# kkrt-labs/stwo-brainfuck

Hardware: AMD Instinct MI355X
Metric: trace cells committed+proved/sec (higher is better)
Workload: dtype u32 (M31 / QM31 modular arithmetic)

## Files before the change

bindings/rust/bfhip_sys.rs:

```rust
#![allow(non_camel_case_types, dead_code)]
use std::ffi::{c_char, c_void};

#[repr(C)] pub struct BfhipCtx { _private: [u8; 0] }
#[repr(C)] pub struct BfhipTrace { _private: [u8; 0] }
#[repr(C)] #[derive(Clone, Copy, Default, Debug, PartialEq, Eq)] pub struct BfhipConventions { pub merkle_node_hash: u32, pub mix_u64: u32, pub logup_mask_order: u32, pub merkle_channel: u32, pub reserved: [u32; 4] }
#[repr(C)] #[derive(Clone, Copy, Debug, PartialEq, Eq)] pub struct BfhipPcsConfig { pub pow_bits: u32, pub log_blowup_factor: u32, pub log_last_layer_degree_bound: u32, pub n_queries: u32, pub reserved: [u32; 4] }
#[repr(C)] #[derive(Clone, Copy, Default, Debug, PartialEq, Eq)] pub struct BfhipCheckReport { pub component: u32, pub log_size: u32, pub n_bad_cells: u64, pub first_bad_cell: u64, pub first_bad_constraint: i32, pub first_bad_value: [u32; 4], pub bad_per_constraint: [u64; 16], pub claimed_sum: [u32; 4], pub reserved: [u32; 3] }
#[repr(C)] pub struct BfhipLocalGroup { _private: [u8; 0] }
#[repr(C)] pub struct BfhipPool { _private: [u8; 0] }

#[link(name = "bfhip")]
extern "C" {
    pub fn bfhip_last_error() -> *const c_char;
    pub fn bfhip_device_count() -> i32;
    pub fn bfhip_device_memory(device_id: i32, free_bytes: *mut u64, total_bytes: *mut u64) -> i32;
    pub fn bfhip_ctx_create(device_id: i32, max_log_domain: u32, out: *mut *mut BfhipCtx) -> i32;
    pub fn bfhip_ctx_destroy(ctx: *mut BfhipCtx) -> i32;
    pub fn bfhip_ctx_sync(ctx: *mut BfhipCtx) -> i32;
    pub fn bfhip_ctx_set_overlap(ctx: *mut BfhipCtx, mask: u32) -> i32;
    pub fn bfhip_ctx_memory(ctx: *mut BfhipCtx, out: *mut u64) -> i32;
    pub fn bfhip_ctx_set_sync_policy(ctx: *mut BfhipCtx, blocking: i32) -> i32;
    pub fn bfhip_ctx_set_mailbox(ctx: *mut BfhipCtx, mode: i32, timeout_ms: u32, test_delay_ms: i32) -> i32;
    pub fn bfhip_ctx_set_conventions(ctx: *mut BfhipCtx, conv: *const BfhipConventions) -> i32;
    pub fn bfhip_ctx_get_conventions(ctx: *mut BfhipCtx, out: *mut BfhipConventions) -> i32;
// ... 7 lines not shown
    pub fn bfhip_twiddles(ctx: *mut BfhipCtx, tw_d: *mut *const u32, itw_d: *mut *const u32, root_log: *mut u32) -> i32;
    pub fn bfhip_interpolate(ctx: *mut BfhipCtx, src_cols_h: *const *mut u32, dst_cols_h: *const *mut u32, n_cols: u32, log_size: u32, replicated: i32) -> i32;
    pub fn bfhip_evaluate(ctx: *mut BfhipCtx, coeff_cols_h: *const *mut u32, dst_cols_h: *const *mut u32, n_cols: u32, log_size: u32, log_eval: u32, replicated: i32) -> i32;
    pub fn bfhip_is_first_coeffs(ctx: *mut BfhipCtx, log_min: u32, log_max: u32, dst_cols_h: *const *mut u32) -> i32;
    pub fn bfhip_broadcast16(ctx: *mut BfhipCtx, rows_d: *const u32, dst_d: *mut u32, n_rows: usize) -> i32;
    pub fn bfhip_bit_reverse(ctx: *mut BfhipCtx, src_d: *const u32, dst_d: *mut u32, log_size: u32) -> i32;
    pub fn bfhip_batch_inverse_m31(ctx: *mut BfhipCtx, src_d: *const u32, dst_d: *mut u32, n: usize) -> i32;
    pub fn bfhip_batch_inverse_qm31(ctx: *mut BfhipCtx, src_d: *const *const u32, dst_d: *const *mut u32, n: usize) -> i32;
    pub fn bfhip_accumulate(ctx: *mut BfhipCtx, dst_d: *mut u32, src_d: *const u32, n: usize) -> i32;
    pub fn bfhip_eval_at_point(ctx: *mut BfhipCtx, coeffs_d: *const u32, log_size: u32, replicated: i32, point_h: *const u32, out_h: *mut u32) -> i32;
    pub fn bfhip_merkle_commit_layer(ctx: *mut BfhipCtx, log_size: u32, prev_layer_d: *const c_void, cols_h: *const *const u32, col_shifts_h: *const u32, n_cols: u32, out_hashes_d: *mut c_void) -> i32;
    pub fn bfhip_merkle_commit_layer_poseidon252(ctx: *mut BfhipCtx, log_size: u32, prev_layer_d: *const c_void, cols_h: *const *const u32, col_shifts_h: *const u32, n_cols: u32, out_hashes_d: *mut c_void) -> i32;
    pub fn bfhip_hades_permutation(ctx: *mut BfhipCtx, in_h: *const u32, out_h: *mut u32) -> i32;
    pub fn bfhip_fold_line(ctx: *mut BfhipCtx, src_d: *const *const u32, dst_d: *const *mut u32, log_size: u32, alpha_h: *const u32) -> i32;
    pub fn bfhip_fold_circle_into_line(ctx: *mut BfhipCtx, dst_d: *const *mut u32, src_d: *const *const u32, log_size: u32, alpha_h: *const u32) -> i32;
    pub fn bfhip_grind(ctx: *mut BfhipCtx, digest_h: *const u8, pow_bits: u32, nonce: *mut u64) -> i32;
    pub fn bfhip_gather(ctx: *mut BfhipCtx, col_d: *const u32, idx_h: *const u64, n: usize, out_h: *mut u32) -> i32;
    pub fn bfhip_component_shape(component: i32, n_main_cols: *mut u32, n_logup_cols: *mut u32, n_constraints: *mut u32) -> i32;
    pub fn bfhip_logup_generate(ctx: *mut BfhipCtx, component: i32, log_size: u32, main_rows_h: *const *const u32, lookup_h: *const u32, out_cols_h: *const *mut u32, claimed_sum_h: *mut u32) -> i32;
    pub fn bfhip_eval_constraints(ctx: *mut BfhipCtx, component: i32, log_size: u32, is_first_d: *const u32, main_lde_h: *const *const u32, main_shifts_h: *const u32, inter_lde_h: *const *const u32, inter_shifts_h: *const u32, lookup_h: *const u32, claimed_sum_h: *const u32, coeffs_h: *const u32, acc_d: *const *mut u32) -> i32;
    pub fn bfhip_check_constraints(ctx: *mut BfhipCtx, component: i32, log_size: u32, main_rows_h: *const *const u32, logup_cols_h: *const *const u32, lookup_h: *const u32, claimed_sum_h: *const u32, out: *mut BfhipCheckReport) -> i32;
    pub fn bfhip_accumulate_quotients(ctx: *mut BfhipCtx, log_size: u32, cols_h: *const *const u32, col_shifts_h: *const u32, n_cols: u32, n_samples_h: *const u32, sample_points_h: *const u32, sample_values_h: *const u32, random_coeff_h: *const u32, out_d: *const *mut u32) -> i32;
    pub fn bfhip_prove_brainfuck(ctx: *mut BfhipCtx, code: *const c_char, input_h: *const u8, n_input: usize, log_max_rows: u32, proof_json: *mut *mut c_char, proof_len: *mut usize, transcript: *mut *mut c_char, phase_seconds: *mut f64) -> i32;
    pub fn bfhip_free_host(p: *mut c_void);
    pub fn bfhip_ctx_last_proof_flags(ctx: *mut BfhipCtx, flags: *mut u32) -> i32;
    pub fn bfhip_local_group_create(count: u32, out: *mut *mut BfhipLocalGroup) -> i32;
    pub fn bfhip_local_group_destroy(group: *mut BfhipLocalGroup) -> i32;
    pub fn bfhip_ctx_join_local_group(ctx: *mut BfhipCtx, group: *mut BfhipLocalGroup, rank: u32) -> i32;
    pub fn bfhip_rccl_unique_id(id: *mut u8) -> i32;
    pub fn bfhip_ctx_join_rccl_group(ctx: *mut BfhipCtx, id: *const u8, rank: u32, count: u32) -> i32;
// ... 40 lines not shown
```

include/bfhip.h:

```cpp
#ifndef BFHIP_H
#define BFHIP_H
#include <stdint.h>
#include <stddef.h>

#ifdef __cplusplus
extern "C" {
#endif

typedef struct bfhip_ctx bfhip_ctx;
typedef struct bfhip_trace bfhip_trace;

enum { BFHIP_MERKLE_STWO_COMPRESS = 0, BFHIP_MERKLE_RFC7693 = 1 };
enum { BFHIP_MIX_U64_COMPRESS = 0, BFHIP_MIX_U64_HASH = 1 };
enum { BFHIP_LOGUP_MASK_CUR_PREV = 0, BFHIP_LOGUP_MASK_PREV_CUR = 1 };
enum { BFHIP_CHANNEL_BLAKE2S = 0, BFHIP_CHANNEL_POSEIDON252 = 1 };
typedef struct bfhip_conventions {
    uint32_t merkle_node_hash;
    uint32_t mix_u64;
    uint32_t logup_mask_order;
    uint32_t merkle_channel;
    uint32_t reserved[4];
} bfhip_conventions;

const char* bfhip_last_error(void);
// ... 37 lines not shown


int32_t bfhip_broadcast16(bfhip_ctx* ctx, const uint32_t* rows_d, uint32_t* dst_d, size_t n_rows);
int32_t bfhip_bit_reverse(bfhip_ctx* ctx, const uint32_t* src_d, uint32_t* dst_d, uint32_t log_size);
int32_t bfhip_batch_inverse_m31(bfhip_ctx* ctx, const uint32_t* src_d, uint32_t* dst_d, size_t n);
int32_t bfhip_batch_inverse_qm31(bfhip_ctx* ctx, const uint32_t* const src_d[4], uint32_t* const dst_d[4], size_t n);
int32_t bfhip_accumulate(bfhip_ctx* ctx, uint32_t* dst_d, const uint32_t* src_d, size_t n);
int32_t bfhip_eval_at_point(bfhip_ctx* ctx, const uint32_t* coeffs_d, uint32_t log_size, int32_t replicated, const uint32_t point_h[8], uint32_t out_h[4]);
int32_t bfhip_merkle_commit_layer(bfhip_ctx* ctx, uint32_t log_size, const void* prev_layer_d, const uint32_t* const* cols_h, const uint32_t* col_shifts_h,
                                  uint32_t n_cols, void* out_hashes_d);
int32_t bfhip_merkle_commit_layer_poseidon252(bfhip_ctx* ctx, uint32_t log_size, const void* prev_layer_d, const uint32_t* const* cols_h,
                                             const uint32_t* col_shifts_h, uint32_t n_cols, void* out_hashes_d);
int32_t bfhip_hades_permutation(bfhip_ctx* ctx, const uint32_t in_h[24], uint32_t out_h[24]);
int32_t bfhip_fold_line(bfhip_ctx* ctx, const uint32_t* const src_d[4], uint32_t* const dst_d[4], uint32_t log_size, const uint32_t alpha_h[4]);
int32_t bfhip_fold_circle_into_line(bfhip_ctx* ctx, uint32_t* const dst_d[4], const uint32_t* const src_d[4], uint32_t log_size, const uint32_t alpha_h[4]);
int32_t bfhip_grind(bfhip_ctx* ctx, const uint8_t digest_h[32], uint32_t pow_bits, uint64_t* nonce);
int32_t bfhip_gather(bfhip_ctx* ctx, const uint32_t* col_d, const uint64_t* idx_h, size_t n, uint32_t* out_h);


int32_t bfhip_component_shape(int32_t component, uint32_t* n_main_cols, uint32_t* n_logup_cols, uint32_t* n_constraints);
int32_t bfhip_logup_generate(bfhip_ctx* ctx, int32_t component, uint32_t log_size, const uint32_t* const* main_rows_h, const uint32_t lookup_h[24],
                             uint32_t* const* out_cols_h, uint32_t claimed_sum_h[4]);
int32_t bfhip_eval_constraints(bfhip_ctx* ctx, int32_t component, uint32_t log_size, const uint32_t* is_first_d, const uint32_t* const* main_lde_h,
                               const uint32_t* main_shifts_h, const uint32_t* const* inter_lde_h, const uint32_t* inter_shifts_h, const uint32_t lookup_h[24],
                               const uint32_t claimed_sum_h[4], const uint32_t* coeffs_h, uint32_t* const acc_d[4]);
typedef struct bfhip_check_report {
    uint32_t component, log_size;
    uint64_t n_bad_cells;
    uint64_t first_bad_cell;
    int32_t  first_bad_constraint;
// ... 86 lines not shown
```

stwo-brainfuck_amd/__init__.py:

```python
import ctypes
import os
import weakref

import numpy as np

_HERE = os.path.dirname(os.path.abspath(__file__))
_LIB_PATH = os.environ.get("BFHIP_LIBRARY") or os.path.join(_HERE, "libbfhip.so")
TESTHOOKS_LIBRARY = os.path.join(_HERE, "libbfhip_testhooks.so")
_lib = None

P = (1 << 31) - 1


class BfhipError(RuntimeError):
    pass


def lib():
    global _lib
    if _lib is None:
        if not os.path.exists(_LIB_PATH):
            raise BfhipError(f"{_LIB_PATH} is missing: build it with __graft_entry__.build(); there is no CPU fallback")
        _lib = ctypes.CDLL(_LIB_PATH)
        _lib.bfhip_last_error.restype = ctypes.c_char_p
# ... 182 lines not shown
        return out

    def set_overlap(self, mask=1):
        _check(lib().bfhip_ctx_set_overlap(self._h, int(mask)))

    def set_sync_policy(self, blocking):
        _check(lib().bfhip_ctx_set_sync_policy(self._h, 1 if blocking else 0))

    def set_mailbox(self, mode=-2, timeout_ms=0, test_delay_ms=-1):
        _check(lib().bfhip_ctx_set_mailbox(self._h, int(mode), int(timeout_ms), int(test_delay_ms)))

    def last_proof_flags(self):
        f = ctypes.c_uint32()
        _check(lib().bfhip_ctx_last_proof_flags(self._h, ctypes.byref(f)))
        return {"mailbox_order": bool(f.value & 1), "kept_preprocessed": bool(f.value & 2), "shared_preprocessed": bool(f.value & 4), "replicated_transforms": bool(f.value & 8),
                "split_gather": bool(f.value & 16)}

    def clock_probe(self, seconds=0.6):
        out = (ctypes.c_double * 6)()
        _check(lib().bfhip_clock_probe(self._h, ctypes.c_double(seconds), out))
        return dict(zip(("ghz", "ghz_min", "ghz_max", "G_compressions_per_s", "launches", "ms_per_launch"), [float(v) for v in out]))

    def clock_probe_mix(self, seconds=0.5, log_nodes=22):
        out = (ctypes.c_double * 6)()
        _check(lib().bfhip_clock_probe_mix(self._h, ctypes.c_double(seconds), int(log_nodes), out))
        d = dict(zip(("ghz", "G_compressions_per_s", "launches", "us_per_launch", "sampler_spanned_the_window", "sampler_seconds"), [float(v) for v in out]))
        d["sampler_spanned_the_window"] = bool(d["sampler_spanned_the_window"])
        return d

    def memory(self):
        out = (ctypes.c_uint64 * 4)()
# ... 104 lines not shown

    def merkle_commit_layer_poseidon252(self, log_size, prev_ptr, col_ptrs, out_ptr, col_shifts=None):
        sh = None if col_shifts is None else (ctypes.c_uint32 * len(col_shifts))(*col_shifts)
        _check(lib().bfhip_merkle_commit_layer_poseidon252(self._h, log_size, ctypes.c_void_p(prev_ptr) if prev_ptr else None, self._ptr_array(col_ptrs), sh, len(col_ptrs), ctypes.c_void_p(out_ptr)))

    def hades_permutation(self, state3):
        words = []
        for x in state3:
            words += [(int(x) >> (32 * i)) & 0xFFFFFFFF for i in range(8)]
        out = (ctypes.c_uint32 * 24)()
        _check(lib().bfhip_hades_permutation(self._h, (ctypes.c_uint32 * 24)(*words), out))
        return [sum(int(out[8 * k + i]) << (32 * i) for i in range(8)) for k in range(3)]

    def fold_line(self, src_ptrs, dst_ptrs, log_size, alpha4):
        _check(lib().bfhip_fold_line(self._h, self._ptr_array(src_ptrs), self._ptr_array(dst_ptrs), log_size, (ctypes.c_uint32 * 4)(*[int(v) for v in alpha4])))

    def fold_circle_into_line(self, dst_ptrs, src_ptrs, log_size, alpha4):
        _check(lib().bfhip_fold_circle_into_line(self._h, self._ptr_array(dst_ptrs), self._ptr_array(src_ptrs), log_size, (ctypes.c_uint32 * 4)(*[int(v) for v in alpha4])))

    def grind(self, digest32, pow_bits):
        nonce = ctypes.c_uint64()
        _check(lib().bfhip_grind(self._h, bytes(digest32), pow_bits, ctypes.byref(nonce)))
        return nonce.value

    def gather(self, col_ptr, indices):
        idx = np.ascontiguousarray(indices, dtype=np.uint64)
        out = np.empty(idx.size, dtype=np.uint32)
        _check(lib().bfhip_gather(self._h, ctypes.c_void_p(col_ptr), idx.ctypes.data_as(ctypes.c_void_p), ctypes.c_size_t(idx.size), out.ctypes.data_as(ctypes.c_void_p)))
        return out

# ... 235 lines not shown
```

stwo-brainfuck_amd/csrc/api.hip:

```cpp
#include "../../include/bfhip.h"
#include "ctx.h"
#include <cstdlib>
#include "host/circle.h"
#include "host/quotients.h"
#include "host/hash.h"
#include <cstdio>
#include <vector>
#include <algorithm>
#include <chrono>

using namespace bf;

static thread_local std::string g_err;
void bfhip_set_error(const std::string& s) { g_err = s; }

#define API_TRY try {
#define API_CTX(ctx) try { if (!(ctx)) throw HipError("null context"); (ctx)->c.bind();
#define API_CATCH } catch (const std::exception& e) { g_err = e.what(); return -1; } catch (...) { g_err = "unknown error"; return -1; }

namespace bf {

void Ctx::ensure_aux() { for (auto& a : aux) if (!a) BF_HIP(hipStreamCreateWithFlags(&a, hipStreamNonBlocking)); }
void Ctx::ensure_side() { if (!stream2) BF_HIP(hipStreamCreateWithFlags(&stream2, hipStreamNonBlocking)); }

// ... 591 lines not shown
    c.stage_checkpoint();
    return c.stage(w, 8);
}
int32_t bfhip_fold_line(bfhip_ctx* ctx, const uint32_t* const src_d[4], uint32_t* const dst_d[4], uint32_t log_size, const uint32_t alpha_h[4]) {
    API_CTX(ctx)
    if (log_size < 1 || log_size > ctx->c.tw_root_log) throw HipError("fold_line: log_size outside the twiddle tree");
    fold_line(ctx->c.stream, dst_d, src_d, stage_alpha(ctx->c, alpha_h), ctx->c.d_itw, ctx->c.tw_root_log, log_size); BF_HIP(hipGetLastError()); return 0;
    API_CATCH
}
int32_t bfhip_fold_circle_into_line(bfhip_ctx* ctx, uint32_t* const dst_d[4], const uint32_t* const src_d[4], uint32_t log_size, const uint32_t alpha_h[4]) {
    API_CTX(ctx)
    if (log_size < 3 || log_size > ctx->c.tw_root_log + 1) throw HipError("fold_circle_into_line: log_size outside the twiddle tree");
    fold_circle_into_line(ctx->c.stream, dst_d, src_d, stage_alpha(ctx->c, alpha_h), ctx->c.d_itw, ctx->c.tw_root_log, log_size); BF_HIP(hipGetLastError()); return 0;
    API_CATCH
}
int32_t bfhip_grind(bfhip_ctx* ctx, const uint8_t digest_h[32], uint32_t pow_bits, uint64_t* nonce) {
    API_CTX(ctx)
    Ctx& c = ctx->c;
    c.stage_checkpoint();
    u32* d_digest = (u32*)c.stage(digest_h, 32);
    unsigned long long init = ~0ull, best = ~0ull;
    unsigned long long* d_best = c.stage(&init, 1);
    const u32 span = 1u << 20;
    for (u64 base = 0; best == ~0ull; base += span) {
        grind_span(c.stream, d_digest, base, span, pow_bits, d_best, c.conv.mix_u64);
        BF_HIP(hipMemcpyAsync(&best, d_best, 8, hipMemcpyDeviceToHost, c.stream));
        c.sync();
        if (base > (u64(1) << 40)) throw HipError("grind: no nonce found below 2^40");
    }
    *nonce = best;
// ... 301 lines not shown
```

stwo-brainfuck_amd/csrc/kernels.h:

```cpp
#pragma once
#include <hip/hip_runtime.h>
#include "m31.h"
#include "air.h"
#include <string>
#include <vector>

struct bfhip_trace;

namespace bf {

struct ColDesc { const u32* ptr; u32 shift; u32 pad_; };

int prof_mode(hipStream_t s);
void prof_enable(hipStream_t s, int mode);
void prof_run_begin(hipStream_t s, const char* name);
void prof_run_end(hipStream_t s);
void prof_begin(hipStream_t s, const char* name, double bytes, double units, double aux = 0.0);
void prof_end(hipStream_t s);
void prof_reset(hipStream_t s);
std::string prof_report_json(const hipStream_t* streams, int n);
void prof_forget(hipStream_t s);
struct ProfScope {
    hipStream_t s; bool on;
    ProfScope(hipStream_t s_, const char* name, double bytes, double units = 0.0, bool dominant = false, double aux = 0.0) : s(s_) {
// ... 70 lines not shown
struct FriTailArgs {
    u32 n_layers, top_log;
    u32 alpha_idx, root_idx;
    u32* ev_last[4];
    u32* chan; u32* alpha; u32* roots;
    const u32* itw; u32 tw_total, rfc;
    FriTailLayer layer[10];
};
void fri_tail(hipStream_t stream, const FriTailArgs* d_args, double bytes, double compressions);
struct FriLayerArgs {
    const u32* src[4]; const u32* quot[4]; u32* dst[4]; uint4* tree[18];
    const u32* alpha8; const u32* itw; u32 tw_total, log, rfc, pad_;
    u32* counter; u32* chan; u32* alpha_out; u32* root_out;
};
void fri_layer(hipStream_t stream, const FriLayerArgs& a);
void grind_span(hipStream_t stream, const u32* d_digest, u64 base, u32 span, u32 pow_bits, unsigned long long* d_best, u32 mix_u64_conv);
void clock_probe_launch(hipStream_t stream, uint4* d_stamps, u32* d_sink, u32 blocks, u32 iters);
void clock_sampler_launch(hipStream_t stream, uint4* d_out, const u32* d_stop_alias, unsigned long long max_ticks);
void fill_mix(hipStream_t stream, u32* p, size_t n);
void channel_mix_root_draw(hipStream_t stream, u32* d_chan, const u32* d_root, u32* d_alpha8, u32* d_root_copy);

void merkle_layer_poseidon(hipStream_t stream, void* out, const void* prev, const ColDesc* d_cols, u32 ncols, u32 log, u32 out_shift = 0, u32 prev_shift = 0,
                           u32 first = 0, u32 count = 0);
void hades_once(hipStream_t stream, const u32* d_in24, u32* d_out24);

struct ConstraintLaunch {
    const u32* is_first; ColDesc trace[13]; ColDesc inter[12]; u32* acc[4]; Q31 coeff[12]; Lookups el; Q31 total_sum; u32 denom_inv[2]; u32 log_size;
    u32 overwrite;
    u32 row0, n_rows;
    const u32* inter_prev[4];
// ... 52 lines not shown
```

stwo-brainfuck_amd/csrc/merkle.hip:

```cpp
#include "kernels.h"
#include <stdexcept>

namespace bf {

__device__ __constant__ const u32 B2S_IV[8] = {0x6A09E667u, 0xBB67AE85u, 0x3C6EF372u, 0xA54FF53Au, 0x510E527Fu, 0x9B05688Cu, 0x1F83D9ABu, 0x5BE0CD19u};

__device__ __forceinline__ u32 rotr(u32 x, int r) { return __builtin_amdgcn_alignbit(x, x, r); }

#define B2S_G(a, b, c, d, x, y) \
    a = a + b + (x); d = rotr(d ^ a, 16); c = c + d; b = rotr(b ^ c, 12); \
    a = a + b + (y); d = rotr(d ^ a, 8);  c = c + d; b = rotr(b ^ c, 7);

#define B2S_ROUND(s0, s1, s2, s3, s4, s5, s6, s7, s8, s9, s10, s11, s12, s13, s14, s15) \
    B2S_G(v0, v4, v8, v12, m[s0], m[s1]) B2S_G(v1, v5, v9, v13, m[s2], m[s3])           \
    B2S_G(v2, v6, v10, v14, m[s4], m[s5]) B2S_G(v3, v7, v11, v15, m[s6], m[s7])         \
    B2S_G(v0, v5, v10, v15, m[s8], m[s9]) B2S_G(v1, v6, v11, v12, m[s10], m[s11])       \
    B2S_G(v2, v7, v8, v13, m[s12], m[s13]) B2S_G(v3, v4, v9, v14, m[s14], m[s15])

__device__ __forceinline__ void blake2s_compress(u32 h[8], const u32 m[16], u32 t0, u32 f0) {
    u32 v0 = h[0], v1 = h[1], v2 = h[2], v3 = h[3], v4 = h[4], v5 = h[5], v6 = h[6], v7 = h[7];
    u32 v8 = 0x6A09E667u, v9 = 0xBB67AE85u, v10 = 0x3C6EF372u, v11 = 0xA54FF53Au;
    u32 v12 = 0x510E527Fu ^ t0, v13 = 0x9B05688Cu, v14 = 0x1F83D9ABu ^ f0, v15 = 0x5BE0CD19u;
    B2S_ROUND(0, 1, 2, 3, 4, 5, 6, 7, 8, 9, 10, 11, 12, 13, 14, 15)
    B2S_ROUND(14, 10, 4, 8, 9, 15, 13, 6, 1, 12, 0, 2, 11, 7, 5, 3)
// ... 123 lines not shown
            for (int k = 0; k < 16; k++) m[k] = k < NC ? nx[k < NC ? k : 0] : 0u;
            st += stride;
            const bool more = st < n_stored;
            i = (first + min(st, n_stored - 1)) << out_shift;
#pragma unroll
            for (int k = 0; k < NC; k++) nx[k] = ld_col(d[k], i);
            u32 h[8];
            blake2s_compress_first<RFC>(h, m, 4u * NC, true);
            store_hash(out, cur, h);
            if (!more) return;
        }
    } else {
        constexpr bool HAS_CHILDREN = SHAPE == MS_INNER0 || SHAPE == MS_INNER_COLS;
        if constexpr (SHAPE == MS_INNER0) ncols = 0;
        for (; st < n_stored; st += stride) merkle_node<RFC, HAS_CHILDREN>(first + st, out, prev, cols, ncols, out_shift, prev_shift);
    }
}

__device__ void channel_step(u32* __restrict__ chan, const u32* __restrict__ root, u32* __restrict__ alpha_out, u32* __restrict__ root_out, u32* alpha_lds = nullptr) {
    u32 h[8], m[16], digest[8];
    for (int k = 0; k < 8; k++) { m[k] = chan[k]; m[8 + k] = root[k]; root_out[k] = root[k]; h[k] = B2S_IV[k]; }
    h[0] ^= 0x01010020u;
    blake2s_compress(h, m, 64, 0xFFFFFFFFu);
    for (int k = 0; k < 8; k++) digest[k] = h[k];
    u32 n_sent = 0;
    for (;;) {
        for (int k = 0; k < 8; k++) { m[k] = digest[k]; m[8 + k] = 0; h[k] = B2S_IV[k]; }
        m[8] = n_sent++;
        h[0] ^= 0x01010020u;
        blake2s_compress(h, m, 64, 0xFFFFFFFFu);
// ... 470 lines not shown
#ifndef MERKLE_NODES_PER_LANE
#define MERKLE_NODES_PER_LANE 4
#endif
void merkle_layer(hipStream_t stream, void* out, const void* prev, const ColDesc* d_cols, u32 ncols, u32 log, double col_bytes, u32 out_shift, u32 prev_shift,
                  u32 node_conv, u32 first, u32 count) {
    const u32 total = (1u << log) >> out_shift;
    const u32 n = count ? count : total;
    u32 threads = n < 256 ? (n < 64 ? 64 : n) : 256;
    const double frac = (double)n / (double)total;
    const double comp_per_node = (prev ? 1.0 : 0.0) + (double)((ncols + 15) / 16) + ((!prev && ncols == 0) ? 1.0 : 0.0);
    ProfScope ps(stream, "k_merkle_layer", ((prev ? 64.0 * total : 0.0) + 32.0 * total + col_bytes) * frac, comp_per_node * n, true);
    u32 blocks = (n + threads - 1) / threads;
    if (blocks >= (1u << 14)) blocks /= MERKLE_NODES_PER_LANE;
    (node_conv ? launch_merkle_layer<true> : launch_merkle_layer<false>)(stream, blocks, threads, (uint4*)out, (const uint4*)prev, d_cols, ncols, n, out_shift, prev_shift, count ? first : 0u);
}
void merkle_subtree(hipStream_t stream, const MerkleTreeDesc& tree, u32 hi, u32 node_conv, double bytes, double compressions) {
    ProfScope ps(stream, "k_merkle_subtree", bytes, compressions);
    hipLaunchKernelGGL(k_merkle_subtree, dim3(1u << MERKLE_SUBTREE_ROOT_LEVEL), dim3(256), 0, stream, tree, hi, node_conv ? 0xFFFFFFFFu : 0u,
                       (u32)MERKLE_SUBTREE_ROOT_LEVEL, (u32)MERKLE_SUBTREE_ROOT_LEVEL, 0u);
}
void merkle_subtree_share(hipStream_t stream, const MerkleTreeDesc& tree, u32 hi, u32 stop, u32 lo, u32 wg0, u32 n_wg, u32 node_conv, double bytes, double compressions) {
    if (hi < stop || stop < lo || hi - lo > 9 || !n_wg) throw std::runtime_error("merkle_subtree_share: bad level range");
    ProfScope ps(stream, "k_merkle_subtree", bytes, compressions);
    hipLaunchKernelGGL(k_merkle_subtree, dim3(n_wg), dim3(256), 0, stream, tree, hi, node_conv ? 0xFFFFFFFFu : 0u, lo, stop, wg0);
}
void merkle_top(hipStream_t stream, const MerkleTreeDesc& tree, u32 top_hi, u32 node_conv, u32* d_chan, u32* d_alpha8, u32* d_root_copy, double bytes, double compressions,
                u32* d_stamp, u32 stamp_value) {
    ProfScope ps(stream, "k_merkle_top", bytes, compressions);
    hipLaunchKernelGGL(k_merkle_top, dim3(1), dim3(256), 0, stream, tree, top_hi, d_chan, d_alpha8, d_root_copy, node_conv ? 0xFFFFFFFFu : 0u, d_stamp, stamp_value);
}
// ... 74 lines not shown
```

stwo-brainfuck_amd/csrc/prover.hip:

```cpp
#include <atomic>
#include "../../include/bfhip.h"
#include "ctx.h"
#include "host/circle.h"
#include "host/quotients.h"
#include "host/proof.h"
#include "host/verifier.h"
#include <map>
#include <set>
#include <chrono>
#include <algorithm>
#include <cstdio>
#include <functional>
#include <mutex>

namespace bf {

void build_tables_device(Ctx& c, const std::vector<u32> trace7_soa[7], u32 n, const std::vector<u32>& code, const std::function<u32*(size_t)>& alloc,
                         std::vector<std::vector<u32*>>& cols_out, u32 log_sizes_out[13]);

static constexpr u32 OWNER_ALL = 0xFFFFFFFFu;

struct DCol {
    u32* ptr = nullptr; u32 log_size = 0; u32 shift = 0;
    u32 lc = 0;
// ... 161 lines not shown
        fft_launch(fft_prepare(inverse, src, dst));
    }

    template <class F> void stage_blocks(Mailbox* mbx, F&& f) {
        if (mbx) { mbx->begin(); f(); mbx->arm(); }
        else { StageBatch sb(c); f(); sb.end(); }
    }

    struct ChannelStep { u32* chan; u32* alpha8; u32* root_copy; };
    struct MerklePlan {
        DevMerkle mk; std::vector<DCol> cols; std::vector<size_t> off; std::vector<double> bytes; size_t n_all = 0;
        const ColDesc* d_all = nullptr; MerkleTreeDesc tree{}; bool poseidon = false;
        u32 fused_top = 0, sub_hi = 0;
        double top_bytes = 0, top_comp = 0, sub_bytes = 0, sub_comp = 0;
        int band_fuse_hi = -1; u32 band_fuse_r = 0; double band_bytes = 0, band_comp = 0;
    };
    MerklePlan merkle_plan(const std::vector<DCol>& cols_in) {
        if (cols_in.empty()) throw HipError("merkle_commit: no columns");
        MerklePlan p;
        p.cols = cols_in;
        std::vector<DCol>& cols = p.cols;
        std::stable_sort(cols.begin(), cols.end(), [](const DCol& a, const DCol& b) { return a.log_size > b.log_size; });
        DevMerkle& mk = p.mk;
        mk.cols = cols;
        mk.max_log = cols[0].log_size;
        mk.layers.resize(mk.max_log + 1);
        mk.shifts.assign(mk.max_log + 1, 0);
        u32 min_col_log = cols.back().log_size;
        std::vector<ColDesc> all; p.off.assign(mk.max_log + 2, 0); p.bytes.assign(mk.max_log + 1, 0.0);
        {
            size_t ci = 0;
            for (int log = (int)mk.max_log; log >= 0; log--) {
// ... 17 lines not shown
            while (lo <= (int)mk.max_log && (int)lo - (int)mk.shifts[lo] < (int)sg.log_count + share_min) lo++;
            const bool worth = (int)mk.max_log - (int)mk.shifts[mk.max_log] >= (int)sg.log_count + (int)SLICE_MIN_LOG_PER_RANK;
            if (worth && lo <= (int)mk.max_log) { mk.band_hi = (int)mk.max_log; mk.band_lo = lo; }
            for (auto& col : cols) if (col.sliced() && ((int)col.log_size < mk.band_lo || (int)col.log_size > mk.band_hi)) throw HipError("shard group: a row-sharded column lies outside the share-wise Merkle band");
        }
        const bool banded = mk.band_hi >= mk.band_lo;
        for (int log = (int)mk.max_log; log >= 0; log--) {
            const size_t stored = (size_t(1) << log) >> mk.shifts[log];
            if (banded && log > mk.band_lo && log <= mk.band_hi) {
                const size_t per_rank = stored >> sg.log_count;
                mk.layers[log] = reinterpret_cast<u32*>(reinterpret_cast<uintptr_t>(c.arena.alloc(32 * per_rank)) - 32 * per_rank * sg.rank);
            } else mk.layers[log] = (u32*)c.arena.alloc(32 * stored);
        }
        if (fused_top == 10 && mk.max_log >= 11) {
            u32 hi = std::min<u32>(banded ? (u32)mk.band_lo - 1 : mk.max_log, 17);
            while (hi > 10 && mk.shifts[hi] != 0) hi--;
            if (hi > 10) { p.sub_hi = hi; p.fused_top = fused_top = MERKLE_SUBTREE_ROOT_LEVEL; }
        }
        auto level_cols = [&](int log) { return (log > 0 ? p.off[log - 1] : all.size()) - p.off[log]; };
        auto level_cost = [&](int log, double& bytes, double& comp) {
            const double nodes = (double)(1u << log), nc = (double)level_cols(log);
            const bool has = log < (int)mk.max_log;
            bytes += nodes * ((has ? 64.0 : 0.0) + 32.0) + p.bytes[log];
            comp += nodes * ((has ? 1.0 : 0.0) + (double)(((u32)nc + 15) / 16) + ((!has && nc == 0) ? 1.0 : 0.0));
        };
        if (banded && !p.poseidon && fused_top > 0 && mk.band_hi > mk.band_lo && c.shard.band_fusion) {
            const int hi = std::min(mk.band_hi, mk.band_lo + 3);
            bool plain = true;
            for (int lg = mk.band_lo; lg <= std::min(hi + 1, (int)mk.max_log); lg++) plain = plain && mk.shifts[lg] == 0;
            const u32 r = 8 - (u32)(hi - mk.band_lo);
            if (plain && (u32)mk.band_lo >= sg.log_count + r) {
                p.band_fuse_hi = hi; p.band_fuse_r = r;
                for (int lg = hi; lg >= mk.band_lo; lg--) level_cost(lg, p.band_bytes, p.band_comp);
                p.band_bytes /= sg.count; p.band_comp /= sg.count;
            }
        }
        for (int log = (int)fused_top - 1; log >= 0; log--) level_cost(log, p.top_bytes, p.top_comp);
        if (p.sub_hi) for (int log = (int)p.sub_hi; log >= (int)MERKLE_SUBTREE_ROOT_LEVEL; log--) level_cost(log, p.sub_bytes, p.sub_comp);
        p.d_all = all.empty() ? nullptr : c.stage(all.data(), all.size());
        if (fused_top > 0) {
            MerkleTreeDesc td{};
            if (mk.max_log >= 32) throw HipError("merkle: tree too deep");
            for (u32 lg = 0; lg <= mk.max_log; lg++) { td.layers[lg] = (uint4*)mk.layers[lg]; td.shifts[lg] = mk.shifts[lg]; td.col_off[lg] = (u32)p.off[lg]; }
            td.cols = p.d_all; td.n_cols = (u32)all.size(); td.max_log = mk.max_log;
            p.tree = td;
        }
        return p;
    }
    struct LevelWait { int level; hipEvent_t ev; };
    DevMerkle merkle_run(MerklePlan& p, Hash32* pinned_root = nullptr, bool no_readback = false, const ChannelStep* step = nullptr, const std::vector<LevelWait>* waits = nullptr,
                         int stamp_slot = -1, bool* stamped = nullptr) {
        DevMerkle& mk = p.mk;
        const ShardGroup& sg = c.shard;
        const bool poseidon = p.poseidon;
// ... 4 lines not shown
        const int single_lo = p.sub_hi ? (int)p.sub_hi + 1 : (int)fused_top;
        size_t wi = 0;
        auto apply_waits = [&](int log) { while (waits && wi < waits->size() && (*waits)[wi].level >= log) BF_HIP(hipStreamWaitEvent(c.stream, (*waits)[wi++].ev, 0)); };
        for (int log = (int)mk.max_log; log >= single_lo; log--) {
            apply_waits(log);
            if (log == p.band_fuse_hi) {
                prof_run_end(c.stream);
                const u32 n_wg = ((1u << mk.band_lo) >> sg.log_count) >> p.band_fuse_r;
                merkle_subtree_share(c.stream, p.tree, (u32)log, (u32)mk.band_lo, (u32)mk.band_lo - p.band_fuse_r, sg.rank * n_wg, n_wg, c.conv.merkle_node_hash, p.band_bytes, p.band_comp);
                sg.comm->all_gather(c.stream, mk.layers[mk.band_lo], (size_t(32) << mk.band_lo) >> sg.log_count);
                prof_run_begin(c.stream, layer_kernel);
                log = mk.band_lo;
                continue;
            }
            size_t n = (log > 0 ? p.off[log - 1] : p.n_all) - p.off[log];
            const bool share = log >= mk.band_lo && log <= mk.band_hi;
            const u32 per_rank = share ? ((1u << (log - mk.shifts[log])) >> sg.log_count) : 0u;
            if (poseidon)
                merkle_layer_poseidon(c.stream, mk.layers[log], log < (int)mk.max_log ? mk.layers[log + 1] : nullptr, n ? p.d_all + p.off[log] : nullptr, (u32)n, (u32)log,
                                      mk.shifts[log], log < (int)mk.max_log ? mk.shifts[log + 1] : 0, sg.rank * per_rank, per_rank);
            else
                merkle_layer(c.stream, mk.layers[log], log < (int)mk.max_log ? mk.layers[log + 1] : nullptr, n ? p.d_all + p.off[log] : nullptr, (u32)n, (u32)log, p.bytes[log],
                             mk.shifts[log], log < (int)mk.max_log ? mk.shifts[log + 1] : 0, c.conv.merkle_node_hash, sg.rank * per_rank, per_rank);
            if (share && log == mk.band_lo) {
                prof_run_end(c.stream);
                sg.comm->all_gather(c.stream, mk.layers[log], ((size_t(32) << log) >> mk.shifts[log]) >> sg.log_count);
                prof_run_begin(c.stream, layer_kernel);
            }
        }
        prof_run_end(c.stream);
// ... 692 lines not shown
        {
            float ms0 = 0.f, ms1 = 0.f;
            if (!reuse) BF_HIP(hipEventElapsedTime(&ms0, c.ev[0], c.ev[1]));
            BF_HIP(hipEventElapsedTime(&ms1, c.ev[0], c.ev[2]));
            const double tot = (double)ms0 + (double)ms1;
            tm.preprocessed = tot > 0 ? wall_phase01 * ms0 / tot : 0.0;
            tm.main_trace = wall_phase01 - tm.preprocessed;
        }
        {
            float ms_q = 0.f;
            BF_HIP(hipEventElapsedTime(&ms_q, c.ev[4], c.ev[5]));
            tm.quotients = ms_q * 1e-3;
            tm.fri = (now() - t0) - tm.quotients;
        }

        c.last_proof_flags = (c.last_proof_flags & 16u) | (mb ? 1u : 0u) | (reuse && !shared ? 2u : 0u) | (shared ? 4u : 0u) | (replicate() ? 8u : 0u);
        tm.total = now() - t_start;
        mark("done");
        print_marks();
        return bp;
    }

    struct CompositionPlan {
        std::vector<ConstraintLaunch> launches; std::vector<DSecure> acc; std::vector<bool> have; u32 total = 0, max_log = 0;
        ConstraintLaunch* h_staged = nullptr;
    };
    CompositionPlan composition_prepare(std::vector<DTree>& trees, const BrainfuckProof& bp, const size_t* main_off, const size_t* inter_off, const Lookups& el) {
        CompositionPlan cp;
        for (int k = 0; k < N_COMPONENTS; k++) { cp.total += n_constraints(k); cp.max_log = std::max(cp.max_log, bp.log_sizes[k] + 1); }
        const bool own_domain = cfg.log_blowup != 1;
        std::vector<DCol> cd_src, cd_dst;
// ... 358 lines not shown
        struct StreamRestore { Ctx& c; hipStream_t s; ~StreamRestore() { c.stream = s; } } restore_stream{c, main_stream};
        BF_HIP(hipMemcpyAsync(d_chan, pinned_chan, 36, hipMemcpyHostToDevice, c.stream));
        const bool host_channel = c.conv.merkle_channel == 1;
        u32 line_log = quotients[0].log_size - 1;
        const u32 last_log = cfg.log_last_layer_degree_bound + cfg.log_blowup;
        if (line_log > last_log + max_layers) throw HipError("FRI: too many layers");
        auto new_layer = [&](u32 log) {
            DSecure l; l.log_size = log; l.lc = slice_log(log) ? lc() : 0;
            for (int w = 0; w < 4; w++) l.c[w] = l.lc ? alloc_slice(log) : c.alloc_u32(size_t(1) << log);
            return l;
        };
        const u32 n_inner = line_log > last_log ? line_log - last_log : 0;
        std::vector<DSecure> layers(n_inner + 1);
        for (u32 i = 0; i <= n_inner; i++) layers[i] = new_layer(line_log - i);
        std::vector<MerklePlan> plans;
        if (!host_channel) {
            c.stage_checkpoint();
            StageBatch sb(c);
            plans.reserve(n_inner + 1);
            plans.push_back(merkle_plan(first_cols));
            for (u32 i = 0; i < n_inner; i++) plans.push_back(merkle_plan(secure_cols(layers[i])));
            sb.end();
        }
        auto commit_step = [&](size_t plan_idx, const std::vector<DCol>& cols, u32 alpha_idx, u32 root_idx) -> DevMerkle {
            if (!host_channel) { ChannelStep st{d_chan, d_alpha + 8 * alpha_idx, d_roots + 8 * root_idx}; return merkle_run(plans[plan_idx], nullptr, true, &st); }
            DevMerkle t = merkle_commit(cols);
            ch.mix_root(t.root);
            const Q31 a = ch.draw_felt(), sq = q_mul(a, a);
            const u32 w[8] = {a.a.a, a.a.b, a.b.a, a.b.b, sq.a.a, sq.a.b, sq.b.a, sq.b.b};
            c.stage_checkpoint();
            const u32* st = c.stage(w, 8);
            BF_HIP(hipMemcpyAsync(d_alpha + 8 * alpha_idx, st, 32, hipMemcpyDeviceToDevice, c.stream));
            return t;
        };
        DevMerkle first_tree;
        if (first_on_aux) {
// ... 4 lines not shown
            c.stream = main_stream;
            BF_HIP(hipStreamWaitEvent(main_stream, e3, 0));
        } else first_tree = commit_step(0, first_cols, 0, 0);
        struct Inner { DSecure ev; DevMerkle tree; };
        std::vector<Inner> inner;
        auto fold_range = [&](u32 src_log, bool src_sliced, u32& first, u32& count) {
            if (src_sliced) { first = (u32)(slice_first(src_log) >> 1); count = (u32)(slice_cells(src_log) >> 1); } else { first = 0; count = 0; }
        };
        auto complete = [&](const DSecure& l) { for (int w = 0; w < 4; w++) c.shard.comm->all_gather(c.stream, l.c[w], sizeof(u32) << (l.log_size - lc())); };
        size_t qi = 0;
        if (quotients[0].log_size - 1 != line_log) throw HipError("FRI: first layer size");
        {
            const DSecure& q = quotients[qi++];
            const u32* src[4] = {q.c[0], q.c[1], q.c[2], q.c[3]};
            u32 first, count; fold_range(q.log_size, q.lc != 0, first, count);
            fold_circle_into_line(c.stream, layers[0].c, src, d_alpha, c.d_itw, c.tw_root_log, q.log_size, true, first, count);
            if (q.lc != 0 && layers[0].lc == 0) complete(layers[0]);
        }
        const u32 TAIL_LOG = 10;
        auto fused = [&](u32 k) { const u32 lg = line_log - k; return !host_channel && k >= 1 && k < n_inner && lg >= 11 && lg <= 16 && layers[k].lc == 0 && layers[k - 1].lc == 0; };
        auto take_quotient = [&](u32 size) -> const DSecure* {
            const DSecure* q = (qi < quotients.size() && quotients[qi].log_size == size) ? &quotients[qi++] : nullptr;
            if (qi < quotients.size() && quotients[qi].log_size == size) throw HipError("FRI: two quotient columns of one size");
            return q;
        };
        u32* d_counter = nullptr;
        u32 li = 0;
        for (; li < n_inner; li++) {
            const u32 log = line_log - li;
            if (!host_channel && log <= TAIL_LOG) break;
            Inner in; in.ev = layers[li];
            if (fused(li)) {
// ... 4 lines not shown
                FriLayerArgs fa{};
                for (int w = 0; w < 4; w++) { fa.src[w] = layers[li - 1].c[w]; fa.quot[w] = q ? q->c[w] : nullptr; fa.dst[w] = layers[li].c[w]; }
                for (u32 lg = 0; lg <= log; lg++) { if (mk.shifts[lg] != 0) throw HipError("FRI layer: replicated level"); fa.tree[lg] = (uint4*)mk.layers[lg]; }
                fa.alpha8 = d_alpha + 8 * li; fa.itw = c.d_itw; fa.tw_total = 1u << c.tw_root_log; fa.log = log; fa.rfc = c.conv.merkle_node_hash ? 0xFFFFFFFFu : 0u;
                fa.counter = d_counter; fa.chan = d_chan; fa.alpha_out = d_alpha + 8 * (li + 1); fa.root_out = d_roots + 8 * (1 + li);
                fri_layer(c.stream, fa);
                in.tree = mk;
            } else in.tree = commit_step(1 + li, secure_cols(layers[li]), li + 1, 1 + li);
            inner.push_back(in);
            if (fused(li + 1)) continue;
            const DSecure* q = take_quotient(log);
            DSecure& next = layers[li + 1];
            const u32* src[4] = {layers[li].c[0], layers[li].c[1], layers[li].c[2], layers[li].c[3]};
            const u32* qs[4] = {q ? q->c[0] : nullptr, q ? q->c[1] : nullptr, q ? q->c[2] : nullptr, q ? q->c[3] : nullptr};
            if (q && (q->lc != 0) != (layers[li].lc != 0)) throw HipError("FRI: a layer and the quotient of its size are sharded differently");
            u32 first, count; fold_range(log, layers[li].lc != 0, first, count);
            fold_line_circle(c.stream, next.c, src, q ? qs : nullptr, d_alpha + 8 * (li + 1), c.d_itw, c.tw_root_log, log, first, count);
            if (layers[li].lc != 0 && next.lc == 0) complete(next);
        }
        if (li < n_inner) {
            FriTailArgs ta{};
            ta.n_layers = n_inner - li; ta.top_log = line_log - li; ta.alpha_idx = li + 1; ta.root_idx = 1 + li;
            ta.chan = d_chan; ta.alpha = d_alpha; ta.roots = d_roots; ta.itw = c.d_itw; ta.tw_total = 1u << c.tw_root_log; ta.rfc = c.conv.merkle_node_hash ? 0xFFFFFFFFu : 0u;
            if (ta.n_layers > 10 || ta.top_log > TAIL_LOG) throw HipError("FRI tail: too many layers");
            for (u32 k = 0; k < ta.n_layers; k++) {
                const u32 log = ta.top_log - k;
                FriTailLayer& L = ta.layer[k];
                for (int w = 0; w < 4; w++) L.ev[w] = layers[li + k].c[w];
                if (qi < quotients.size() && quotients[qi].log_size == log) { for (int w = 0; w < 4; w++) L.quot[w] = quotients[qi].c[w]; qi++; }
                const DevMerkle& mk = plans[1 + li + k].mk;
// ... 387 lines not shown
```

Baseline: 14.27 billion.

## Fuse FRI fold with Merkle leaf hashing for large layers

Adds a kernel that folds the previous FRI layer (line, circle, or line plus circle quotient) and immediately Blake2s-hashes each folded row as a Merkle leaf, writing both the folded values and the leaf hashes. For single-device runs with layers of log size 17 and above, the separate fold launch is skipped and the fold is described to the Merkle plan, which runs the fused kernel in place of the deepest-level leaf launch. This removes one full write-then-reread of each folded layer and one kernel launch per layer. In exchange the Merkle plan gets extra constraints: the subtree fusion cannot cover the deepest level, and certain tree shapes now throw.

```diff
diff --git a/bindings/rust/bfhip_sys.rs b/bindings/rust/bfhip_sys.rs
--- a/bindings/rust/bfhip_sys.rs
+++ b/bindings/rust/bfhip_sys.rs
@@ -45,6 +45,7 @@
     pub fn bfhip_hades_permutation(ctx: *mut BfhipCtx, in_h: *const u32, out_h: *mut u32) -> i32;
     pub fn bfhip_fold_line(ctx: *mut BfhipCtx, src_d: *const *const u32, dst_d: *const *mut u32, log_size: u32, alpha_h: *const u32) -> i32;
     pub fn bfhip_fold_circle_into_line(ctx: *mut BfhipCtx, dst_d: *const *mut u32, src_d: *const *const u32, log_size: u32, alpha_h: *const u32) -> i32;
+    pub fn bfhip_fri_fold_leaf(ctx: *mut BfhipCtx, src_d: *const *const u32, quot_d: *const *const u32, dst_d: *const *mut u32, log_size: u32, alpha_h: *const u32, out_hashes_d: *mut c_void) -> i32;
     pub fn bfhip_grind(ctx: *mut BfhipCtx, digest_h: *const u8, pow_bits: u32, nonce: *mut u64) -> i32;
     pub fn bfhip_gather(ctx: *mut BfhipCtx, col_d: *const u32, idx_h: *const u64, n: usize, out_h: *mut u32) -> i32;
     pub fn bfhip_component_shape(component: i32, n_main_cols: *mut u32, n_logup_cols: *mut u32, n_constraints: *mut u32) -> i32;
diff --git a/include/bfhip.h b/include/bfhip.h
--- a/include/bfhip.h
+++ b/include/bfhip.h
@@ -75,6 +75,8 @@
 int32_t bfhip_hades_permutation(bfhip_ctx* ctx, const uint32_t in_h[24], uint32_t out_h[24]);
 int32_t bfhip_fold_line(bfhip_ctx* ctx, const uint32_t* const src_d[4], uint32_t* const dst_d[4], uint32_t log_size, const uint32_t alpha_h[4]);
 int32_t bfhip_fold_circle_into_line(bfhip_ctx* ctx, uint32_t* const dst_d[4], const uint32_t* const src_d[4], uint32_t log_size, const uint32_t alpha_h[4]);
+int32_t bfhip_fri_fold_leaf(bfhip_ctx* ctx, const uint32_t* const src_d[4], const uint32_t* const quot_d[4], uint32_t* const dst_d[4], uint32_t log_size,
+                            const uint32_t alpha_h[4], void* out_hashes_d);
 int32_t bfhip_grind(bfhip_ctx* ctx, const uint8_t digest_h[32], uint32_t pow_bits, uint64_t* nonce);
 int32_t bfhip_gather(bfhip_ctx* ctx, const uint32_t* col_d, const uint64_t* idx_h, size_t n, uint32_t* out_h);
 
diff --git a/stwo-brainfuck_amd/__init__.py b/stwo-brainfuck_amd/__init__.py
--- a/stwo-brainfuck_amd/__init__.py
+++ b/stwo-brainfuck_amd/__init__.py
@@ -220,7 +220,7 @@
         f = ctypes.c_uint32()
         _check(lib().bfhip_ctx_last_proof_flags(self._h, ctypes.byref(f)))
         return {"mailbox_order": bool(f.value & 1), "kept_preprocessed": bool(f.value & 2), "shared_preprocessed": bool(f.value & 4), "replicated_transforms": bool(f.value & 8),
-                "split_gather": bool(f.value & 16)}
+                "split_gather": bool(f.value & 16), "fri_fold_leaf": bool(f.value & 32)}
 
     def clock_probe(self, seconds=0.6):
         out = (ctypes.c_double * 6)()
@@ -355,6 +355,10 @@
 
     def fold_line(self, src_ptrs, dst_ptrs, log_size, alpha4):
         _check(lib().bfhip_fold_line(self._h, self._ptr_array(src_ptrs), self._ptr_array(dst_ptrs), log_size, (ctypes.c_uint32 * 4)(*[int(v) for v in alpha4])))
+
+    def fri_fold_leaf(self, src_ptrs, quot_ptrs, dst_ptrs, log_size, alpha4, out_ptr):
+        _check(lib().bfhip_fri_fold_leaf(self._h, self._ptr_array(src_ptrs) if src_ptrs is not None else None, self._ptr_array(quot_ptrs) if quot_ptrs is not None else None,
+                                         self._ptr_array(dst_ptrs), log_size, (ctypes.c_uint32 * 4)(*[int(v) for v in alpha4]), ctypes.c_void_p(out_ptr)))
 
     def fold_circle_into_line(self, dst_ptrs, src_ptrs, log_size, alpha4):
         _check(lib().bfhip_fold_circle_into_line(self._h, self._ptr_array(dst_ptrs), self._ptr_array(src_ptrs), log_size, (ctypes.c_uint32 * 4)(*[int(v) for v in alpha4])))
diff --git a/stwo-brainfuck_amd/csrc/api.hip b/stwo-brainfuck_amd/csrc/api.hip
--- a/stwo-brainfuck_amd/csrc/api.hip
+++ b/stwo-brainfuck_amd/csrc/api.hip
@@ -629,6 +629,21 @@
     fold_circle_into_line(ctx->c.stream, dst_d, src_d, stage_alpha(ctx->c, alpha_h), ctx->c.d_itw, ctx->c.tw_root_log, log_size); BF_HIP(hipGetLastError()); return 0;
     API_CATCH
 }
+int32_t bfhip_fri_fold_leaf(bfhip_ctx* ctx, const uint32_t* const src_d[4], const uint32_t* const quot_d[4], uint32_t* const dst_d[4], uint32_t log_size,
+                            const uint32_t alpha_h[4], void* out_hashes_d) {
+    API_CTX(ctx)
+    Ctx& c = ctx->c;
+    if (!src_d && !quot_d) throw HipError("fri_fold_leaf: neither a line source nor a circle evaluation");
+    if (!dst_d || !alpha_h || !out_hashes_d) throw HipError("fri_fold_leaf: null argument");
+    if (log_size < 2 || log_size + 1 > c.tw_root_log + (src_d ? 0u : 1u)) throw HipError("fri_fold_leaf: log_size outside the twiddle tree");
+    FriFoldLeafArgs fa{};
+    for (int w = 0; w < 4; w++) { fa.src[w] = src_d ? src_d[w] : nullptr; fa.quot[w] = quot_d ? quot_d[w] : nullptr; fa.dst[w] = dst_d[w]; }
+    fa.alpha8 = stage_alpha(c, alpha_h); fa.itw = c.d_itw; fa.tw_total = 1u << c.tw_root_log; fa.log = log_size;
+    fri_fold_leaf(c.stream, out_hashes_d, fa, !src_d ? FF_CIRCLE : quot_d ? FF_LINE_CIRCLE : FF_LINE, c.conv.merkle_node_hash);
+    BF_HIP(hipGetLastError());
+    return 0;
+    API_CATCH
+}
 int32_t bfhip_grind(bfhip_ctx* ctx, const uint8_t digest_h[32], uint32_t pow_bits, uint64_t* nonce) {
     API_CTX(ctx)
     Ctx& c = ctx->c;
diff --git a/stwo-brainfuck_amd/csrc/kernels.h b/stwo-brainfuck_amd/csrc/kernels.h
--- a/stwo-brainfuck_amd/csrc/kernels.h
+++ b/stwo-brainfuck_amd/csrc/kernels.h
@@ -108,6 +108,9 @@
     u32* counter; u32* chan; u32* alpha_out; u32* root_out;
 };
 void fri_layer(hipStream_t stream, const FriLayerArgs& a);
+enum FriFoldMode : int { FF_LINE = 0, FF_LINE_CIRCLE = 1, FF_CIRCLE = 2 };
+struct FriFoldLeafArgs { const u32* src[4]; const u32* quot[4]; u32* dst[4]; const u32* alpha8; const u32* itw; u32 tw_total, log; };
+void fri_fold_leaf(hipStream_t stream, void* out, const FriFoldLeafArgs& a, int mode, u32 node_conv);
 void grind_span(hipStream_t stream, const u32* d_digest, u64 base, u32 span, u32 pow_bits, unsigned long long* d_best, u32 mix_u64_conv);
 void clock_probe_launch(hipStream_t stream, uint4* d_stamps, u32* d_sink, u32 blocks, u32 iters);
 void clock_sampler_launch(hipStream_t stream, uint4* d_out, const u32* d_stop_alias, unsigned long long max_ticks);
diff --git a/stwo-brainfuck_amd/csrc/merkle.hip b/stwo-brainfuck_amd/csrc/merkle.hip
--- a/stwo-brainfuck_amd/csrc/merkle.hip
+++ b/stwo-brainfuck_amd/csrc/merkle.hip
@@ -161,6 +161,66 @@
         constexpr bool HAS_CHILDREN = SHAPE == MS_INNER0 || SHAPE == MS_INNER_COLS;
         if constexpr (SHAPE == MS_INNER0) ncols = 0;
         for (; st < n_stored; st += stride) merkle_node<RFC, HAS_CHILDREN>(first + st, out, prev, cols, ncols, out_shift, prev_shift);
+    }
+}
+
+struct FriFoldIn { uint2 s[4]; u32 xinv; uint2 q[4]; u32 cx, cy; };
+template <int MODE>
+__device__ __forceinline__ void fri_fold_load(FriFoldIn& in, const FriFoldLeafArgs& a, u32 i) {
+    if constexpr (MODE != FF_CIRCLE) {
+        in.xinv = a.itw[a.tw_total - (2u << a.log) + i];
+#pragma unroll
+        for (int w = 0; w < 4; w++) in.s[w] = reinterpret_cast<const uint2*>(a.src[w])[i];
+    }
+    if constexpr (MODE != FF_LINE) {
+        const u32* t1 = a.itw + (a.tw_total - (1u << a.log));
+        in.cx = t1[(i >> 2) * 2]; in.cy = t1[(i >> 2) * 2 + 1];
+#pragma unroll
+        for (int w = 0; w < 4; w++) in.q[w] = reinterpret_cast<const uint2*>(a.quot[w])[i];
+    }
+}
+template <int MODE>
+__device__ __forceinline__ Q31 fri_fold_row(const FriFoldIn& in, u32 i, const QConst& k_alpha, const QConst& k_alpha_sq) {
+    Q31 r = q_make(0, 0, 0, 0);
+    if constexpr (MODE != FF_CIRCLE) {
+        const Q31 fx = q_make(in.s[0].x, in.s[1].x, in.s[2].x, in.s[3].x), fn = q_make(in.s[0].y, in.s[1].y, in.s[2].y, in.s[3].y);
+        r = q_add(q_add(fx, fn), q_mul_const(q_mulm(q_sub(fx, fn), in.xinv), k_alpha));
+    }
+    if constexpr (MODE != FF_LINE) {
+        const u32 cx = in.cx, cy = in.cy, sel = i & 3;
+        const u32 yinv = sel == 0 ? cy : sel == 1 ? m_neg(cy) : sel == 2 ? m_neg(cx) : cx;
+        const Q31 fp = q_make(in.q[0].x, in.q[1].x, in.q[2].x, in.q[3].x), fn = q_make(in.q[0].y, in.q[1].y, in.q[2].y, in.q[3].y);
+        const Q31 fprime = q_add(q_mul_const(q_mulm(q_sub(fp, fn), yinv), k_alpha), q_add(fp, fn));
+        r = MODE == FF_CIRCLE ? fprime : q_add(q_mul_const(r, k_alpha_sq), fprime);
+    }
+    return r;
+}
+template <bool RFC, int MODE>
+__global__ void __launch_bounds__(256) k_fri_fold_leaf(uint4* __restrict__ out, const FriFoldLeafArgs a) {
+    const u32 stride = gridDim.x * blockDim.x, n = 1u << a.log;
+    u32 st = blockIdx.x * blockDim.x + threadIdx.x;
+    if (st >= n) return;
+    u32 al[8];
+#pragma unroll
+    for (int k = 0; k < 8; k++) al[k] = ld_constant(a.alpha8 + k);
+    const QConst k_alpha = q_const(q_make(al[0], al[1], al[2], al[3])), k_alpha_sq = q_const(q_make(al[4], al[5], al[6], al[7]));
+    FriFoldIn nx;
+    fri_fold_load<MODE>(nx, a, st);
+    for (;;) {
+        const u32 cur = st;
+        const Q31 r = fri_fold_row<MODE>(nx, cur, k_alpha, k_alpha_sq);
+        st += stride;
+        const bool more = st < n;
+        fri_fold_load<MODE>(nx, a, min(st, n - 1));
+        u32 m[16];
+#pragma unroll
+        for (int k = 4; k < 16; k++) m[k] = 0u;
+        m[0] = r.a.a; m[1] = r.a.b; m[2] = r.b.a; m[3] = r.b.b;
+        a.dst[0][cur] = m[0]; a.dst[1][cur] = m[1]; a.dst[2][cur] = m[2]; a.dst[3][cur] = m[3];
+        u32 h[8];
+        blake2s_compress_first<RFC>(h, m, 16u, true);
+        store_hash(out, cur, h);
+        if (!more) return;
     }
 }
 
@@ -661,6 +721,22 @@
     if (blocks >= (1u << 14)) blocks /= MERKLE_NODES_PER_LANE;
     (node_conv ? launch_merkle_layer<true> : launch_merkle_layer<false>)(stream, blocks, threads, (uint4*)out, (const uint4*)prev, d_cols, ncols, n, out_shift, prev_shift, count ? first : 0u);
 }
+template <bool RFC>
+static void launch_fri_fold_leaf(hipStream_t stream, u32 blocks, u32 threads, uint4* out, const FriFoldLeafArgs& a, int mode) {
+    auto* k = mode == FF_LINE ? k_fri_fold_leaf<RFC, FF_LINE> : mode == FF_LINE_CIRCLE ? k_fri_fold_leaf<RFC, FF_LINE_CIRCLE> : k_fri_fold_leaf<RFC, FF_CIRCLE>;
+    hipLaunchKernelGGL(k, dim3(blocks), dim3(threads), 0, stream, out, a);
+}
+void fri_fold_leaf(hipStream_t stream, void* out, const FriFoldLeafArgs& a, int mode, u32 node_conv) {
+    if (mode != FF_LINE && mode != FF_LINE_CIRCLE && mode != FF_CIRCLE) throw std::runtime_error("fri_fold_leaf: unknown mode");
+    if (a.log > 29) throw std::runtime_error("fri_fold_leaf: layer too large");
+    const u32 n = 1u << a.log;
+    const u32 threads = n < 256 ? (n < 64 ? 64 : n) : 256;
+    const double per_row = 32.0 + 16.0 + (mode != FF_CIRCLE ? 32.0 + 4.0 : 0.0) + (mode != FF_LINE ? 32.0 + 2.0 : 0.0);
+    ProfScope ps(stream, "k_merkle_layer", per_row * n, (double)n, true);
+    u32 blocks = (n + threads - 1) / threads;
+    if (blocks >= (1u << 14)) blocks /= MERKLE_NODES_PER_LANE;
+    (node_conv ? launch_fri_fold_leaf<true> : launch_fri_fold_leaf<false>)(stream, blocks, threads, (uint4*)out, a, mode);
+}
 void merkle_subtree(hipStream_t stream, const MerkleTreeDesc& tree, u32 hi, u32 node_conv, double bytes, double compressions) {
     ProfScope ps(stream, "k_merkle_subtree", bytes, compressions);
     hipLaunchKernelGGL(k_merkle_subtree, dim3(1u << MERKLE_SUBTREE_ROOT_LEVEL), dim3(256), 0, stream, tree, hi, node_conv ? 0xFFFFFFFFu : 0u,
diff --git a/stwo-brainfuck_amd/csrc/prover.hip b/stwo-brainfuck_amd/csrc/prover.hip
--- a/stwo-brainfuck_amd/csrc/prover.hip
+++ b/stwo-brainfuck_amd/csrc/prover.hip
@@ -199,8 +199,9 @@
         u32 fused_top = 0, sub_hi = 0;
         double top_bytes = 0, top_comp = 0, sub_bytes = 0, sub_comp = 0;
         int band_fuse_hi = -1; u32 band_fuse_r = 0; double band_bytes = 0, band_comp = 0;
+        bool folded_leaves = false; FriFoldLeafArgs fold{}; int fold_mode = -1;
     };
-    MerklePlan merkle_plan(const std::vector<DCol>& cols_in) {
+    MerklePlan merkle_plan(const std::vector<DCol>& cols_in, bool folded_leaves = false) {
         if (cols_in.empty()) throw HipError("merkle_commit: no columns");
         MerklePlan p;
         p.cols = cols_in;
@@ -248,6 +249,7 @@
         }
         if (fused_top == 10 && mk.max_log >= 11) {
             u32 hi = std::min<u32>(banded ? (u32)mk.band_lo - 1 : mk.max_log, 17);
+            if (folded_leaves && hi == mk.max_log) hi--;
             while (hi > 10 && mk.shifts[hi] != 0) hi--;
             if (hi > 10) { p.sub_hi = hi; p.fused_top = fused_top = MERKLE_SUBTREE_ROOT_LEVEL; }
         }
@@ -272,6 +274,11 @@
         for (int log = (int)fused_top - 1; log >= 0; log--) level_cost(log, p.top_bytes, p.top_comp);
         if (p.sub_hi) for (int log = (int)p.sub_hi; log >= (int)MERKLE_SUBTREE_ROOT_LEVEL; log--) level_cost(log, p.sub_bytes, p.sub_comp);
         p.d_all = all.empty() ? nullptr : c.stage(all.data(), all.size());
+        if (folded_leaves) {
+            if (banded || p.poseidon || mk.shifts[mk.max_log] != 0 || level_cols((int)mk.max_log) != 4 || (int)mk.max_log < (p.sub_hi ? (int)p.sub_hi + 1 : (int)fused_top))
+                throw HipError("merkle_plan: this tree's deepest level cannot be a fused fold + leaf launch");
+            p.folded_leaves = true;
+        }
         if (fused_top > 0) {
             MerkleTreeDesc td{};
             if (mk.max_log >= 32) throw HipError("merkle: tree too deep");
@@ -306,6 +313,12 @@
                 continue;
             }
             size_t n = (log > 0 ? p.off[log - 1] : p.n_all) - p.off[log];
+            if (p.folded_leaves && log == (int)mk.max_log) {
+                if (p.fold_mode < 0 || p.fold.log != mk.max_log) throw HipError("merkle_run: the fold of the deepest level was not described");
+                fri_fold_leaf(c.stream, mk.layers[log], p.fold, p.fold_mode, c.conv.merkle_node_hash);
+                c.last_proof_flags |= 32u;
+                continue;
+            }
             const bool share = log >= mk.band_lo && log <= mk.band_hi;
             const u32 per_rank = share ? ((1u << (log - mk.shifts[log])) >> sg.log_count) : 0u;
             if (poseidon)
@@ -1028,7 +1041,7 @@
             tm.fri = (now() - t0) - tm.quotients;
         }
 
-        c.last_proof_flags = (c.last_proof_flags & 16u) | (mb ? 1u : 0u) | (reuse && !shared ? 2u : 0u) | (shared ? 4u : 0u) | (replicate() ? 8u : 0u);
+        c.last_proof_flags = (c.last_proof_flags & 48u) | (mb ? 1u : 0u) | (reuse && !shared ? 2u : 0u) | (shared ? 4u : 0u) | (replicate() ? 8u : 0u);
         tm.total = now() - t_start;
         mark("done");
         print_marks();
@@ -1417,12 +1430,22 @@
         std::vector<DSecure> layers(n_inner + 1);
         for (u32 i = 0; i <= n_inner; i++) layers[i] = new_layer(line_log - i);
         std::vector<MerklePlan> plans;
+        auto fold_leaf = [&](u32 k) {
+            return !host_channel && c.shard.count == 1 && k < n_inner && line_log - k >= 17 && layers[k].lc == 0 && (k == 0 ? quotients[0].lc == 0 : layers[k - 1].lc == 0);
+        };
+        auto describe_fold = [&](u32 k, const DSecure* src, const DSecure* q) {
+            MerklePlan& p = plans[1 + k];
+            FriFoldLeafArgs& fa = p.fold;
+            for (int w = 0; w < 4; w++) { fa.src[w] = src ? src->c[w] : nullptr; fa.quot[w] = q ? q->c[w] : nullptr; fa.dst[w] = layers[k].c[w]; }
+            fa.alpha8 = d_alpha + 8 * k; fa.itw = c.d_itw; fa.tw_total = 1u << c.tw_root_log; fa.log = line_log - k;
+            p.fold_mode = !src ? FF_CIRCLE : q ? FF_LINE_CIRCLE : FF_LINE;
+        };
         if (!host_channel) {
             c.stage_checkpoint();
             StageBatch sb(c);
             plans.reserve(n_inner + 1);
             plans.push_back(merkle_plan(first_cols));
-            for (u32 i = 0; i < n_inner; i++) plans.push_back(merkle_plan(secure_cols(layers[i])));
+            for (u32 i = 0; i < n_inner; i++) plans.push_back(merkle_plan(secure_cols(layers[i]), fold_leaf(i)));
             sb.end();
         }
         auto commit_step = [&](size_t plan_idx, const std::vector<DCol>& cols, u32 alpha_idx, u32 root_idx) -> DevMerkle {
@@ -1457,8 +1480,11 @@
             const DSecure& q = quotients[qi++];
             const u32* src[4] = {q.c[0], q.c[1], q.c[2], q.c[3]};
             u32 first, count; fold_range(q.log_size, q.lc != 0, first, count);
-            fold_circle_into_line(c.stream, layers[0].c, src, d_alpha, c.d_itw, c.tw_root_log, q.log_size, true, first, count);
-            if (q.lc != 0 && layers[0].lc == 0) complete(layers[0]);
+            if (fold_leaf(0)) describe_fold(0, nullptr, &q);
+            else {
+                fold_circle_into_line(c.stream, layers[0].c, src, d_alpha, c.d_itw, c.tw_root_log, q.log_size, true, first, count);
+                if (q.lc != 0 && layers[0].lc == 0) complete(layers[0]);
+            }
         }
         const u32 TAIL_LOG = 10;
         auto fused = [&](u32 k) { const u32 lg = line_log - k; return !host_channel && k >= 1 && k < n_inner && lg >= 11 && lg <= 16 && layers[k].lc == 0 && layers[k - 1].lc == 0; };
@@ -1493,6 +1519,7 @@
             const u32* src[4] = {layers[li].c[0], layers[li].c[1], layers[li].c[2], layers[li].c[3]};
             const u32* qs[4] = {q ? q->c[0] : nullptr, q ? q->c[1] : nullptr, q ? q->c[2] : nullptr, q ? q->c[3] : nullptr};
             if (q && (q->lc != 0) != (layers[li].lc != 0)) throw HipError("FRI: a layer and the quotient of its size are sharded differently");
+            if (fold_leaf(li + 1)) { describe_fold(li + 1, &layers[li], q); continue; }
             u32 first, count; fold_range(log, layers[li].lc != 0, first, count);
             fold_line_circle(c.stream, next.c, src, q ? qs : nullptr, d_alpha + 8 * (li + 1), c.d_itw, c.tw_root_log, log, first, count);
             if (layers[li].lc != 0 && next.lc == 0) complete(next);
```

Result: faster. 14.43 billion (median of 6 runs) (+1.1%).
